# Ewenwan/ORB-YGZ-SLAM

Hardware: AMD Instinct MI355X
Metric: frames/sec ORB-extract+SparseImageAlign, 752x480, 1000 feat (higher is better)
Workload: dtype u8; 1 GPU; C5 offline sequence: 13728 frames (EuRoC MH01..05 length) sharded over 1 GPU(s), per frame C2 extract + dense Hamming (k vs k-1) + C3 SparseImgAlign levels 3..1, device-packed result slots gathered to rank 0 over RCCL; sequence_frames=13728, frames_per_gpu=13728, frames_extracted_per_gpu=13731, chunks=4, image=752x480, nfeatures=1000, nlevels=4, align_pairs_per_gpu=13727, parallelism=frame-sharded x1 (contiguous shards + 1-frame halo), collective=none (N=1: rank 0 is the root), schedule=pipe, hip_graph=False

## Files before the change

orb-ygz-slam_amd/csrc/api_batch.cpp:

```cpp
#include "host.hpp"

namespace ygzfe {
int batch_wait(ygzfe_batch *b) {
    YGZ_HIP(hipStreamSynchronize(b->stream));
    if (b->desc_pending) YGZ_HIP(hipEventSynchronize(b->ev_desc_done));
    return YGZFE_OK;
}
}

static const char *kStageNames[] = {"pyramid", "blur7", "fast9_cells", "octree", "orient_rbrief", "hamming_best2",
                                    "sparse_align", "stereo", "pack_slots"};
constexpr int kNumStages = 9;

extern "C" {

int ygzfe_batch_create(const ygzfe_orb_params *p, int device, int width, int height, int max_frames,
                       ygzfe_batch **out) {
    if (!p || !out || max_frames <= 0) { set_error("invalid argument"); return YGZFE_EINVAL; }
    YGZ_TRY(ensure_device(device));
    std::unique_ptr<ygzfe_batch> b(new ygzfe_batch());
    b->p = *p;
    b->device = device;
    b->maxF = max_frames;
    YGZ_TRY(make_plan(*p, width, height, &b->plan));
    const Plan &P = b->plan->hp();
    YGZ_TRY(b->pyr.ensure((size_t)max_frames * P.pyr_bytes));
    YGZ_TRY(b->ws.ensure(P, max_frames, P.kp_cap));
    YGZ_HIP(hipMemset(b->ws.err.p, 0, 16));
    YGZ_HIP(hipStreamCreateWithFlags(&b->stream, hipStreamNonBlocking));
    for (int i = 0; i < 3; i++) {
        YGZ_HIP(hipStreamCreateWithFlags(&b->aux[i], hipStreamNonBlocking));
        YGZ_HIP(hipEventCreateWithFlags(&b->ev_join[i], hipEventDisableTiming));
    }
    YGZ_HIP(hipEventCreateWithFlags(&b->ev_fork, hipEventDisableTiming));
    YGZ_HIP(hipEventCreateWithFlags(&b->ev_oct_fork, hipEventDisableTiming));
    YGZ_HIP(hipEventCreateWithFlags(&b->ev_desc_done, hipEventDisableTiming));
    for (int i = 0; i < 2; i++) YGZ_HIP(hipEventCreateWithFlags(&b->ev_oct_join[i], hipEventDisableTiming));
    *out = b.release();
    return YGZFE_OK;
}
// ... 41 lines not shown
    YGZ_HIP(hipStreamSynchronize(b->stream));
    if (d_pyramids) b->pyr.bind(d_pyramids, (size_t)b->maxF * P.pyr_bytes);
    if (d_kps) b->ws.kps.bind(d_kps, (size_t)b->maxF * P.kp_cap * sizeof(ygzfe_kp));
    if (d_desc) b->ws.desc.bind(d_desc, (size_t)b->maxF * P.kp_cap * 32);
    if (d_counts) b->ws.counts.bind(d_counts, (size_t)b->maxF * 4);
    return YGZFE_OK;
}

int ygzfe_batch_upload(ygzfe_batch *b, const uint8_t *frames, int n_frames) {
    if (!b || !frames || n_frames < 0 || n_frames > b->maxF) { set_error("invalid argument"); return YGZFE_EINVAL; }
    YGZ_TRY(ensure_device(b->device));
    const Plan &P = b->plan->hp();
    if (b->desc_pending) YGZ_HIP(hipStreamWaitEvent(b->stream, b->ev_desc_done, 0));
    YGZ_HIP(hipMemcpy2DAsync(b->pyr.p, P.pyr_bytes, frames, (size_t)P.W * P.H, (size_t)P.W * P.H, n_frames,
                             hipMemcpyHostToDevice, b->stream));
    YGZ_HIP(hipStreamSynchronize(b->stream));
    return YGZFE_OK;
}

int ygzfe_batch_extract_split(ygzfe_batch *b, int n_frames, void *kp_stream, void *desc_stream) {
    if (!b || n_frames < 0 || n_frames > b->maxF) { set_error("invalid argument"); return YGZFE_EINVAL; }
    if (n_frames == 0) return YGZFE_OK;
    YGZ_TRY(ensure_device(b->device));
    hipStream_t st = kp_stream ? (hipStream_t)kp_stream : b->stream;
    hipStream_t ds = desc_stream ? (hipStream_t)desc_stream : st;
    const PlanDev &pd = *b->plan;
    const Plan &P = pd.hp();
    Workspace &ws = b->ws;
    uint8_t *pyr = b->pyr.as<uint8_t>();
    hipStreamCaptureStatus cap = hipStreamCaptureStatusNone;
    YGZ_HIP(hipStreamIsCapturing(st, &cap));
    if (b->desc_pending && cap == hipStreamCaptureStatusNone) YGZ_HIP(hipStreamWaitEvent(st, b->ev_desc_done, 0));
    YGZ_HIP(hipMemsetAsync(ws.err.p, 0, 16, st));
    static const bool unfused = getenv("YGZFE_PYR_UNFUSED") != nullptr;
    const bool fused = !unfused && pyramid_fusable(P) > 0;
    hipEvent_t t0 = b->begin(st);
    if (fused)
        YGZ_HIP(launch_pyramid_blur0(pyr, ws.blur.as<uint8_t>(), P.pyr_bytes, P, pd.dp(), n_frames, st));
    else
        YGZ_HIP(launch_pyramid(pyr, P.pyr_bytes, P, pd.dp(), pd.tabs.as<int>(), n_frames, st));
    b->end(ST_PYR, t0, st);
    hipStream_t bs = ds;
    if (ds != st) {
        YGZ_HIP(hipEventRecord(b->ev_fork, st));
        YGZ_HIP(hipStreamWaitEvent(ds, b->ev_fork, 0));
    }
    t0 = b->begin(bs);
    if (fused)
        YGZ_HIP(launch_blur_rest(pyr, ws.blur.as<uint8_t>(), P.pyr_bytes, P, pd.dp(), n_frames, bs));
    else
        YGZ_HIP(launch_blur(pyr, ws.blur.as<uint8_t>(), P.pyr_bytes, P, pd.dp(), n_frames, bs));
    b->end(ST_BLUR, t0, bs);
    t0 = b->begin(st);
    YGZ_HIP(launch_fast(pyr, P.pyr_bytes, P, pd.dp(), pd.cells.as<CellDesc>(), ws.cellbuf.as<uint32_t>(),
                        ws.cellcnt.as<int>(), n_frames, st));
    b->end(ST_FAST, t0, st);
    t0 = b->begin(st);
    YGZ_HIP(launch_octree(P, pd.dp(), ws.cellbuf.as<uint32_t>(), ws.cellcnt.as<int>(), ws.candA.as<uint32_t>(),
                          ws.candB.as<uint32_t>(), ws.sel.as<uint32_t>(), ws.selcnt.as<int>(), ws.err.as<int>(),
                          ws.octq.as<int>(),
                          n_frames, st, &b->aux[1], 2, b->ev_oct_fork, b->ev_oct_join));
    YGZ_HIP(launch_emit_kps(P, pd.dp(), ws.sel.as<uint32_t>(), ws.selcnt.as<int>(), nullptr, ws.kps.as<ygzfe_kp>(),
                            ws.counts.as<int>(), P.kp_cap, ws.ojobs.as<uint2>(), n_frames, st));
    b->end(ST_OCT, t0, st);
    if (ds != st) {
        YGZ_HIP(hipEventRecord(b->ev_join[1], st));
        YGZ_HIP(hipStreamWaitEvent(ds, b->ev_join[1], 0));
    }
    t0 = b->begin(ds);
    YGZ_HIP(launch_orient_desc(pyr, ws.blur.as<uint8_t>(), P.pyr_bytes, P, pd.dp(), ws.ojobs.as<uint2>(), nullptr,
                               ws.kps.as<ygzfe_kp>(), ws.desc.as<uint8_t>(), P.kp_cap, n_frames, ds));
    b->end(ST_DESC, t0, ds);
    if (cap == hipStreamCaptureStatusNone) {
        YGZ_HIP(hipEventRecord(b->ev_desc_done, ds));
        b->desc_pending = true;
    }
    return YGZFE_OK;
}

int ygzfe_batch_extract(ygzfe_batch *b, int n_frames, void *stream) {
    return ygzfe_batch_extract_split(b, n_frames, stream, stream);
}

int ygzfe_diag_stage_ms(ygzfe_batch *b, int stage, int n_frames, int reps, int build_pyramid, float *ms) {
    if (!b || !ms || n_frames < 1 || n_frames > b->maxF || reps < 1 || stage < 0 || stage > 2) {
// ... 58 lines not shown
}

int ygzfe_batch_device_results(ygzfe_batch *b, ygzfe_kp **d_kps, uint8_t **d_desc, int32_t **d_counts,
                               int *kp_cap) {
    if (!b) { set_error("null batch"); return YGZFE_EINVAL; }
    if (d_kps) *d_kps = b->ws.kps.as<ygzfe_kp>();
    if (d_desc) *d_desc = b->ws.desc.as<uint8_t>();
    if (d_counts) *d_counts = b->ws.counts.as<int32_t>();
    if (kp_cap) *kp_cap = b->plan->hp().kp_cap;
    return YGZFE_OK;
}

int ygzfe_batch_level(ygzfe_batch *b, int frame, int level, const uint8_t **d_level, int *w, int *h, int *stride) {
    if (!b || frame < 0 || frame >= b->maxF) { set_error("invalid argument"); return YGZFE_EINVAL; }
    const Plan &P = b->plan->hp();
    if (level < 0 || level >= P.nlevels) { set_error("level out of range"); return YGZFE_EINVAL; }
    if (d_level) *d_level = b->pyr.as<uint8_t>() + (size_t)frame * P.pyr_bytes + P.lv[level].off;
    if (w) *w = P.lv[level].w;
    if (h) *h = P.lv[level].h;
    if (stride) *stride = P.lv[level].w;
    return YGZFE_OK;
}

int ygzfe_batch_read_level(ygzfe_batch *b, int frame, int level, int blurred, uint8_t *dst, int dst_stride) {
    if (!b || !dst || frame < 0 || frame >= b->maxF) { set_error("invalid argument"); return YGZFE_EINVAL; }
    const Plan &P = b->plan->hp();
    if (level < 0 || level >= P.nlevels) { set_error("level out of range"); return YGZFE_EINVAL; }
    const LevelDesc &L = P.lv[level];
    if (dst_stride < L.w) { set_error("dst_stride < level width"); return YGZFE_EINVAL; }
    const DevBuf &src = blurred ? b->ws.blur : b->pyr;
    if (!src.p) { set_error("no %s buffer yet (run ygzfe_batch_extract first)", blurred ? "blurred" : "pyramid"); return YGZFE_EINVAL; }
    YGZ_TRY(ensure_device(b->device));
    YGZ_TRY(batch_wait(b));
    YGZ_HIP(hipMemcpy2D(dst, dst_stride, (const uint8_t *)src.p + (size_t)frame * P.pyr_bytes + L.off, L.w, L.w, L.h,
                        hipMemcpyDeviceToHost));
    return YGZFE_OK;
}

int ygzfe_batch_stats(ygzfe_batch *b, int n_frames, int64_t *candidates, int64_t *selected) {
    if (!b || n_frames < 0 || n_frames > b->maxF) { set_error("invalid argument"); return YGZFE_EINVAL; }
    const Plan &P = b->plan->hp();
    YGZ_TRY(ensure_device(b->device));
    YGZ_TRY(batch_wait(b));
    for (int l = 0; l < P.nlevels; l++) {
        if (candidates) candidates[l] = 0;
        if (selected) selected[l] = 0;
    }
    if (n_frames == 0 || !b->ws.cellcnt.p) return YGZFE_OK;
    std::vector<int> cc((size_t)n_frames * P.ncells), sc((size_t)n_frames * P.nlevels);
    if (P.ncells) YGZ_HIP(hipMemcpy(cc.data(), b->ws.cellcnt.p, cc.size() * 4, hipMemcpyDeviceToHost));
    YGZ_HIP(hipMemcpy(sc.data(), b->ws.selcnt.p, sc.size() * 4, hipMemcpyDeviceToHost));
    for (int f = 0; f < n_frames; f++)
        for (int l = 0; l < P.nlevels; l++) {
            const LevelDesc &L = P.lv[l];
            if (candidates)
                for (int c = 0; c < L.ncells; c++) candidates[l] += cc[(size_t)f * P.ncells + L.cell_begin + c];
            if (selected) selected[l] += sc[(size_t)f * P.nlevels + l];
        }
    return YGZFE_OK;
}

int ygzfe_batch_timing(ygzfe_batch *b, int enable, float *ms, const char **names, int cap) {
    if (!b) { set_error("null batch"); return YGZFE_EINVAL; }
    YGZ_TRY(ensure_device(b->device));
    YGZ_TRY(b->collect());
    for (int s = 0; s < kNumStages && s < cap; s++) {
// ... 42 lines not shown
```

orb-ygz-slam_amd/csrc/common.hpp:

```cpp
#pragma once

#include <hip/hip_runtime.h>
#include <stdint.h>

#include "../../include/ygzfe.h"

namespace ygzfe {

constexpr int kMaxLevels = YGZFE_MAX_LEVELS;
#ifndef YGZ_BLUR_ROWS
#define YGZ_BLUR_ROWS 32
#endif
constexpr int kBlurRows = YGZ_BLUR_ROWS;
constexpr int kEdgeThreshold = 19;
constexpr int kMinBorder = kEdgeThreshold - 3;
constexpr int kPatchSize = 31, kHalfPatch = 15;
constexpr int kMaxRoi = 72;

struct LevelDesc {
    int w, h;
    uint32_t off;
    int budget;
    int patch_size;
    float scale, inv_scale;
    int cell_begin, ncells;
    int max_bx, max_by;
    int n_ini;
    float hX;
    int sel_off, sel_cap;
    int cand_off, cand_cap;
    int resize_mode;
    int xtab_off, ytab_off;
    int xmax;
    int blur_tile_begin, blur_tiles_x, blur_tiles_y;
    int pyr_tile_begin;
    int fast_roi;
    int fast_rw, fast_rh;
    int oct_rb, oct_dn, oct_xtab, oct_ytab;
};

struct alignas(16) CellDesc {
    int16_t x0, y0, rw, rh;
    int16_t offx, offy;
    int16_t level, pad;
};

struct Plan {
    int W, H, nlevels;
    uint32_t pyr_bytes;
    int ncells;
    int cell_cap;
    int sel_total;
    int cand_total;
    int kp_cap;
    int ini_th, min_th;
    int blur_variant;
    int blur_tiles;
    int node_cap;
    int fast_S;
    int umax[16];
    LevelDesc lv[kMaxLevels];
    const int32_t *dtabs;
};


template <class T>
using gptr_t = const __attribute__((address_space(1))) T *;
template <class T>
__device__ __forceinline__ gptr_t<T> as_global(const T *p) {
    return (gptr_t<T>)p;
}
template <class T>
using gmut_t = __attribute__((address_space(1))) T *;
template <class T>
__device__ __forceinline__ gmut_t<T> as_global_mut(T *p) {
    return (gmut_t<T>)p;
}
__device__ __forceinline__ uint32_t mad24(uint32_t a, uint32_t b, uint32_t c) {
    uint32_t d;
    asm volatile("v_mad_u32_u24 %0, %1, %2, %3" : "=v"(d) : "v"(a), "v"(b), "v"(c));
    return d;
}

template <class T>
using cptr_t = const __attribute__((address_space(4))) T *;
template <class T>
__device__ __forceinline__ T scalar_load(const T *p) {
    static_assert(sizeof(T) % 4 == 0, "scalar_load: dword-sized records only");
    struct W { uint32_t d[sizeof(T) / 4]; };
    return __builtin_bit_cast(T, *(cptr_t<W>)p);
// ... 180 lines not shown
```

orb-ygz-slam_amd/csrc/extract.hip:

```cpp
#include "common.hpp"

#include <algorithm>
#include <type_traits>

#include "plan.hpp"

namespace ygzfe {

__constant__ __attribute__((aligned(16))) int8_t c_pattern[1024];
__constant__ __attribute__((aligned(16))) uint8_t c_pattern_f8[1024];

#ifdef YGZ_STAMPS
__device__ unsigned long long g_bstamps[1 << 20];
extern "C" int ygzfe_diag_block_stamps(unsigned long long *out, int n) {
    (void)hipDeviceSynchronize();
    (void)hipMemcpyFromSymbol(out, HIP_SYMBOL(g_bstamps), sizeof(unsigned long long) * (size_t)n);
    return 0;
}
#endif


__global__ __launch_bounds__(256) void k_resize_area2(uint8_t *__restrict__ pyr, uint32_t pitch,
                                                      const Plan *__restrict__ plan, int l) {
    const LevelDesc &S = plan->lv[l - 1];
// ... 236 lines not shown
    uint32_t prev;
    uint32_t l1;
    uint32_t l2;
};
#define YGZ_PYR_FUSED_ROW(P, raw, yy, x, store_lane, rs)                                                          \
    do {                                                                                                          \
        if ((yy) & 1) {                                                                                           \
            const uint32_t a_ = __builtin_amdgcn_udot4((raw), 0x00000101u, __builtin_amdgcn_udot4((P).prev, 0x00000101u, 2u, false), false) >> 2; \
            const uint32_t b_ = __builtin_amdgcn_udot4((raw), 0x01010000u, __builtin_amdgcn_udot4((P).prev, 0x01010000u, 2u, false), false) >> 2; \
            if (store_lane)                                                                                       \
                __builtin_amdgcn_raw_buffer_store_b16((uint16_t)(a_ | (b_ << 8)), (rs),                            \
                    (P).off[1] + ((uint32_t)(yy) >> 1) * (P).w[1] + ((uint32_t)(x) >> 1), 0, 0);                   \
            if ((P).K >= 2 && ((yy) & 3) == 3) {                                                                  \
                const uint32_t l2_ = ((P).l1 & 0xFFu) + ((P).l1 >> 8) + a_ + b_ + 2u;                             \
                const uint32_t v2_ = l2_ >> 2;                                                                    \
                if (store_lane)                                                                                   \
                    __builtin_amdgcn_raw_buffer_store_b8((uint8_t)v2_, (rs),                                       \
                        (P).off[2] + ((uint32_t)(yy) >> 2) * (P).w[2] + ((uint32_t)(x) >> 2), 0, 0);               \
                if ((P).K >= 3 && ((yy) & 7) == 7) {                                                              \
                    const uint32_t t_ = (P).l2 + v2_;                                                             \
                    const uint32_t n_ = (uint32_t)__builtin_amdgcn_update_dpp(0, (int)t_, 0xB1, 0xF, 0xF, false); \
                    if ((store_lane) && ((x) & 7) == 0)                                                           \
                        __builtin_amdgcn_raw_buffer_store_b8((uint8_t)((t_ + n_ + 2u) >> 2), (rs),                 \
                            (P).off[3] + ((uint32_t)(yy) >> 3) * (P).w[3] + ((uint32_t)(x) >> 3), 0, 0);           \
                }                                                                                                 \
                (P).l2 = v2_;                                                                                     \
            }                                                                                                     \
            (P).l1 = a_ | (b_ << 8);                                                                              \
        } else {                                                                                                  \
            (P).prev = (raw);                                                                                     \
        }                                                                                                         \
    } while (0)

template <bool CV3, bool PYR>
__device__ __forceinline__ void blur_strip_aligned(const uint8_t *__restrict__ src, uint8_t *__restrict__ dst, int w,
                                                   int hgt, int sx, int y0, int lane, PyrFused &pf) {
    typedef unsigned short u16x2 __attribute__((ext_vector_type(2)));
    constexpr uint32_t k0 = 18, k1 = 34, k2 = CV3 ? 49 : 48, k3 = CV3 ? 55 : 56;
    const int x = sx + 4 * lane;
    const bool left_edge = sx == 0, right_edge = sx + 256 >= w;
    const uint32_t nbytes = (uint32_t)w * (uint32_t)hgt;
    const __amdgpu_buffer_rsrc_t rin = __builtin_amdgcn_make_buffer_rsrc((void *)src, 0, (int)nbytes, 0x00020000);
    const __amdgpu_buffer_rsrc_t rout = __builtin_amdgcn_make_buffer_rsrc((void *)dst, 0, (int)nbytes, 0x00020000);
    const uint32_t voff = (uint32_t)x;
    const uint32_t hoff = lane == 0 ? voff - 4u : voff + 4u;
    constexpr uint32_t K00 = k0 | (k1 << 8) | (k2 << 16) | (k3 << 24), K10 = k2 | (k1 << 8) | (k0 << 16);
    constexpr uint32_t K01 = K00 << 8, K11 = k3 | (k2 << 8) | (k1 << 16) | (k0 << 24);
    constexpr uint32_t K02 = (k0 << 16) | (k1 << 24), K12 = k2 | (k3 << 8) | (k2 << 16) | (k1 << 24), K22 = k0;
    constexpr uint32_t K03 = k0 << 24, K13 = k1 | (k2 << 8) | (k3 << 16) | (k2 << 24), K23 = k1 | (k0 << 8);
    const u16x2 V01 = {(unsigned short)k0, (unsigned short)k1}, V23 = {(unsigned short)k2, (unsigned short)k3};
    const u16x2 V21 = {(unsigned short)k2, (unsigned short)k1};
    struct Row {
        uint32_t a, halo;
    };
    auto fetch = [&](int r, Row &R) {
        const uint32_t so = (uint32_t)(reflect101(y0 + r - 3, hgt) * w);
        R.a = __builtin_amdgcn_raw_buffer_load_b32(rin, voff, so, 0);
        R.halo = __builtin_amdgcn_raw_buffer_load_b32(rin, hoff, so, 0);
    };
    Row buf[kBlurAhead];
#pragma unroll
    for (int r = 0; r < kBlurAhead; r++) fetch(r, buf[r]);
    const bool fix_r = right_edge && x == w;
    const bool fix_halo = right_edge && lane == 63 && w == sx + 256;
    const bool store_lane = x < w;
    uint32_t prv[4] = {0u, 0u, 0u, 0u};
    uint32_t pr[5][4];
    const __amdgpu_buffer_rsrc_t rpyr =
        __builtin_amdgcn_make_buffer_rsrc((void *)pf.frame, 0, PYR ? (int)(pf.off[pf.K] + pf.w[pf.K] * (uint32_t)(hgt >> pf.K)) : 0,
                                          0x00020000);
#pragma unroll
    for (int r = 0; r < kBlurRows + 6; r++) {
        Row cur = buf[r % kBlurAhead];
        if (r + kBlurAhead < kBlurRows + 6) fetch(r + kBlurAhead, buf[r % kBlurAhead]);
        if (PYR && r >= 3 && r < kBlurRows + 3 && y0 + r - 3 < hgt) {
            const int yy = y0 + r - 3;
            YGZ_PYR_FUSED_ROW(pf, cur.a, yy, x, store_lane, rpyr);
        }
        uint32_t am1 = (uint32_t)__builtin_amdgcn_update_dpp((int)cur.halo, (int)cur.a, 0x138, 0xF, 0xF, false);
        if (right_edge) {
            if (fix_r) cur.a = __builtin_amdgcn_perm(cur.a, am1, 0x03000102u);
            if (fix_halo) cur.halo = __builtin_amdgcn_perm(cur.halo, cur.a, 0x03000102u);
        }
        const uint32_t ap1 = (uint32_t)__builtin_amdgcn_update_dpp((int)cur.halo, (int)cur.a, 0x130, 0xF, 0xF, false);
        if (left_edge && lane == 0) am1 = __builtin_amdgcn_perm(ap1, cur.a, 0x01020304u);
        const uint32_t p0 = __builtin_amdgcn_alignbyte(cur.a, am1, 1), p1 = __builtin_amdgcn_alignbyte(ap1, cur.a, 1);
        const uint32_t p2 = ap1 >> 8;
        uint32_t hs[4];
        hs[0] = __builtin_amdgcn_udot4(p1, K10, __builtin_amdgcn_udot4(p0, K00, 0u, false), false);
        hs[1] = __builtin_amdgcn_udot4(p1, K11, __builtin_amdgcn_udot4(p0, K01, 0u, false), false);
        hs[2] = __builtin_amdgcn_udot4(
            p2, K22, __builtin_amdgcn_udot4(p1, K12, __builtin_amdgcn_udot4(p0, K02, 0u, false), false), false);
        hs[3] = __builtin_amdgcn_udot4(
            p2, K23, __builtin_amdgcn_udot4(p1, K13, __builtin_amdgcn_udot4(p0, K03, 0u, false), false), false);
        const int y = y0 + r - 6;
        if (r >= 6 && y < hgt && store_lane) {
            uint32_t pk = 0;
#pragma unroll
            for (int j = 0; j < 4; j++) {
                uint32_t acc = __builtin_amdgcn_udot2(__builtin_bit_cast(u16x2, pr[0][j]), V01, 32768u, false);
                acc = __builtin_amdgcn_udot2(__builtin_bit_cast(u16x2, pr[2][j]), V23, acc, false);
                acc = __builtin_amdgcn_udot2(__builtin_bit_cast(u16x2, pr[4][j]), V21, acc, false);
                uint32_t v = (__umul24(k0, hs[j]) + acc) >> 16;
                if (CV3) v = min(v, 255u);
                pk |= v << (8 * j);
            }
            __builtin_amdgcn_raw_buffer_store_b32(pk, rout, voff, (uint32_t)(y * w), 0);
        }
#pragma unroll
        for (int j = 0; j < 4; j++) {
#pragma unroll
            for (int m = 0; m < 4; m++) pr[m][j] = pr[m + 1][j];
            pr[4][j] = prv[j] | (hs[j] << 16);
            prv[j] = hs[j];
        }
    }
}

#ifndef YGZ_BLUR_EU
#define YGZ_BLUR_EU 7
#endif
#if YGZ_BLUR_EU > 0
#define YGZ_BLUR_ATTR __attribute__((amdgpu_waves_per_eu(YGZ_BLUR_EU)))
#else
#define YGZ_BLUR_ATTR
#endif
template <bool PYR>
__global__ __launch_bounds__(256) YGZ_BLUR_ATTR void k_blur7(uint8_t *__restrict__ pyr,
                                               uint8_t *__restrict__ blur, uint32_t pitch,
                                               const Plan *__restrict__ plan, int task_begin, int task_end,
                                               int pyr_k) {
#ifndef YGZ_BLUR_SWZ
#define YGZ_BLUR_SWZ 1
#endif
    int bx = blockIdx.x, f = blockIdx.y;
    if (YGZ_BLUR_SWZ) swizzled_block_2d(bx, f);
    const int lane = threadIdx.x & 63;
    int task = __builtin_amdgcn_readfirstlane(task_begin + bx * 4 + (threadIdx.x >> 6)), l = 0;
    if (task >= task_end) return;
    while (l + 1 < plan->nlevels && task >= plan->lv[l + 1].blur_tile_begin) l++;
// ... 67 lines not shown
                ring[6][j] = hs[j];
            }
            const int y = y0 + r - 6;
            if (r >= 6 && y < hgt && active) {
                uint32_t pk = 0;
#pragma unroll
                for (int j = 0; j < 4; j++) {
                    const uint32_t acc = __umul24(k0, ring[0][j] + ring[6][j]) + __umul24(k1, ring[1][j] + ring[5][j]) +
                                         __umul24(k2, ring[2][j] + ring[4][j]) + __umul24(k3, ring[3][j]) + 32768u;
                    pk |= min(acc >> 16, 255u) << (8 * j);
                }
                uint8_t *o = dst + (size_t)y * w + x;
                if (x >= 4 && x + 4 <= w - 3 && (((uintptr_t)o) & 3u) == 0) {
                    *reinterpret_cast<uint32_t *>(o) = pk;
                } else {
#pragma unroll
                    for (int j = 0; j < 4; j++)
                        if (x + j >= 4 && x + j < w - 3) o[j] = (uint8_t)(pk >> (8 * j));
                }
            }
        }
    }
    const int ncol = w >= 16 ? 7 : w;
    const bool left = sx == 0, right = sx + 256 >= w;
    if (w >= 16 && !left && !right) return;
    const int nrows = min(kBlurRows, hgt - y0);
    for (int t = lane; t < ncol * nrows; t += 64) {
        const int cidx = t % ncol, r = t / ncol;
        const int xc = w >= 16 ? (cidx < 4 ? cidx : w - 7 + cidx) : cidx;
        if (w >= 16 && ((xc < 4 && !left) || (xc >= w - 3 && !right))) continue;
        const int y = y0 + r;
        dst[(size_t)y * w + xc] = blur_pixel_reflect(src, w, hgt, xc, y, kk);
    }
}


__device__ __forceinline__ int wave_incl_scan(int v) {
    v += __builtin_amdgcn_update_dpp(0, v, 0x111, 0xF, 0xF, false);
    v += __builtin_amdgcn_update_dpp(0, v, 0x112, 0xF, 0xF, false);
    v += __builtin_amdgcn_update_dpp(0, v, 0x114, 0xF, 0xF, false);
    v += __builtin_amdgcn_update_dpp(0, v, 0x118, 0xF, 0xF, false);
    v += __builtin_amdgcn_update_dpp(0, v, 0x142, 0xA, 0xF, false);
    v += __builtin_amdgcn_update_dpp(0, v, 0x143, 0xC, 0xF, false);
    return v;
}

template <int NT>
__device__ __forceinline__ int block_excl_scan(int v, int *red, int *total) {
    const int lane = threadIdx.x & 63, w = threadIdx.x >> 6;
    const int incl = wave_incl_scan(v);
    if (lane == 63) red[w] = incl;
    __syncthreads();
    int off = 0, tot = 0;
#pragma unroll
    for (int i = 0; i < NT / 64; i++) {
        const int r = red[i];
        off += i < w ? r : 0;
        tot += r;
    }
    __syncthreads();
    *total = tot;
    return off + incl - v;
}


template <int S>
// ... 1596 lines not shown
    }
    for (int l = K + 1; l < hp.nlevels; l++) {
        const LevelDesc &D = hp.lv[l];
        dim3 grid((D.w + 63) / 64, (D.h + 3) / 4, nframes);
        if (D.resize_mode == 1)
            hipLaunchKernelGGL(k_resize_area2, grid, dim3(256), 0, st, pyr, pitch, dp, l);
        else
            hipLaunchKernelGGL(k_resize_linear, grid, dim3(256), 0, st, pyr, pitch, dp, dtabs, l);
    }
    return hipGetLastError();
}

hipError_t launch_blur(const uint8_t *pyr, uint8_t *blur, uint32_t pitch, const Plan &hp, const Plan *dp,
                       int nframes, hipStream_t st) {
    hipLaunchKernelGGL(k_blur7<false>, dim3((hp.blur_tiles + 3) / 4, nframes), dim3(256), 0, st,
                       const_cast<uint8_t *>(pyr), blur, pitch, dp, 0, hp.blur_tiles, 0);
    return hipGetLastError();
}

int pyramid_fusable(const Plan &hp) {
    const int K = hp.nlevels - 1;
    if (K < 1 || K > 3 || hp.lv[0].w < 16 || (hp.lv[0].w & 3) || kBlurRows % 8) return 0;
    for (int l = 1; l <= K; l++)
        if (hp.lv[l].resize_mode != 1) return 0;
    return K;
}

hipError_t launch_pyramid_blur0(uint8_t *pyr, uint8_t *blur, uint32_t pitch, const Plan &hp, const Plan *dp,
                                int nframes, hipStream_t st_l0) {
    const int K = pyramid_fusable(hp), n0 = hp.lv[0].blur_tiles_x * hp.lv[0].blur_tiles_y;
    hipLaunchKernelGGL(k_blur7<true>, dim3((n0 + 3) / 4, nframes), dim3(256), 0, st_l0, pyr, blur, pitch, dp, 0, n0, K);
    return hipGetLastError();
}
hipError_t launch_blur_rest(const uint8_t *pyr, uint8_t *blur, uint32_t pitch, const Plan &hp, const Plan *dp,
                            int nframes, hipStream_t st) {
    const int n0 = hp.lv[0].blur_tiles_x * hp.lv[0].blur_tiles_y, n = hp.blur_tiles - n0;
    if (n <= 0) return hipSuccess;
    hipLaunchKernelGGL(k_blur7<false>, dim3((n + 3) / 4, nframes), dim3(256), 0, st, const_cast<uint8_t *>(pyr), blur,
                       pitch, dp, n0, hp.blur_tiles, 0);
    return hipGetLastError();
}

void fast_shape_pick(int rw, int rh, int &S, int &R) {
    fast_slice_shape(rw, rh, S, R);
    if (S == 36 && R > 40) S = 40;
    if (!((S == 36 && R == 40) || (S == 40 && R <= 56))) S = R = std::max(S, R);
}
#define YGZ_FAST_SHAPES(X) X(36, 40) X(40, 40) X(40, 48) X(40, 56) X(48, 48) X(56, 56) X(64, 64) X(72, 72)

hipError_t launch_fast(const uint8_t *pyr, uint32_t pitch, const Plan &hp, const Plan *dp, const CellDesc *dcells,
                       uint32_t *cellbuf, int *cellcnt, int nframes, hipStream_t st0, const hipStream_t *lvl_streams,
                       int n_lvl_streams) {
    if (hp.ncells == 0) return hipSuccess;
    for (int l = 0; l < hp.nlevels; l++) {
        const LevelDesc &L = hp.lv[l];
        if (L.ncells == 0) continue;
        int S, R;
        fast_shape_pick(L.fast_rw, L.fast_rh, S, R);
        const hipStream_t st = (l == 0 || !lvl_streams || n_lvl_streams <= 0) ? st0
                                                                                : lvl_streams[(l - 1) % n_lvl_streams];
#ifndef YGZ_FAST_LDS_MIN
#define YGZ_FAST_LDS_MIN 0
#endif
        const size_t lds = std::max<size_t>(kFastWaves * (size_t)fast_slice_bytes(S, R), YGZ_FAST_LDS_MIN);
        const dim3 grid((L.ncells + kFastWaves - 1) / kFastWaves, nframes);
#define YGZ_FAST(SS, RR)                                                                                        \
    if (S == SS && R == RR)                                                                                     \
        hipLaunchKernelGGL((k_fast_cells<SS, RR>), grid, dim3(64 * kFastWaves), lds, st, pyr, pitch, dp, dcells, \
                           cellbuf, cellcnt, L.cell_begin, L.cell_begin + L.ncells, l, nullptr);
        YGZ_FAST_SHAPES(YGZ_FAST)
#undef YGZ_FAST
    }
// ... 175 lines not shown
```

orb-ygz-slam_amd/csrc/kernels.hpp:

```cpp
#pragma once
#include "common.hpp"

namespace ygzfe {

hipError_t upload_pattern(const int *pat);
hipError_t run_arith_guard(uint32_t host_fails[2]);
hipError_t launch_pyramid(uint8_t *pyr, uint32_t pitch, const Plan &hp, const Plan *dp, const int *dtabs,
                          int nframes, hipStream_t st);
int pyramid_fusable(const Plan &hp);
hipError_t launch_pyramid_blur0(uint8_t *pyr, uint8_t *blur, uint32_t pitch, const Plan &hp, const Plan *dp,
                                int nframes, hipStream_t st_l0);
hipError_t launch_blur_rest(const uint8_t *pyr, uint8_t *blur, uint32_t pitch, const Plan &hp, const Plan *dp,
                            int nframes, hipStream_t st);
hipError_t launch_blur(const uint8_t *pyr, uint8_t *blur, uint32_t pitch, const Plan &hp, const Plan *dp,
                       int nframes, hipStream_t st);
hipError_t launch_fast(const uint8_t *pyr, uint32_t pitch, const Plan &hp, const Plan *dp, const CellDesc *dcells,
                       uint32_t *cellbuf, int *cellcnt, int nframes, hipStream_t st,
                       const hipStream_t *lvl_streams = nullptr, int n_lvl_streams = 0);
hipError_t launch_fast_merged(const uint8_t *pyr, uint32_t pitch, const Plan &hp, const Plan *dp,
                              const CellDesc *dcells, uint32_t *cellbuf, int *cellcnt, int nframes, hipStream_t st,
                              int *clear_flag = nullptr);
hipError_t launch_octree(const Plan &hp, const Plan *dp, const uint32_t *cellbuf, const int *cellcnt,
                         uint32_t *candA, uint32_t *candB, uint32_t *sel, int *selcnt, int *err, int *octq,
                         int nframes, hipStream_t st, const hipStream_t *side = nullptr, int nside = 0,
                         hipEvent_t fork = nullptr, const hipEvent_t *join = nullptr, bool wide = false);
size_t octree_queue_ints(const Plan &hp, int nframes);
void fast_shape_pick(int rw, int rh, int &S, int &R);
void fast_shape_merged(const Plan &hp, int &S, int &R);
int octree_nc(const LevelDesc &L);
int octree_sort0_keys(int nc, bool wide);
int octree_groups(const Plan &hp);
hipError_t launch_emit_kps(const Plan &hp, const Plan *dp, const uint32_t *sel, const int *selcnt,
                           const int *n_existing, ygzfe_kp *kps, int *counts, int row_cap, uint2 *ojobs, int nframes,
                           hipStream_t st);
hipError_t launch_orient_desc(const uint8_t *pyr, const uint8_t *blur, uint32_t pitch, const Plan &hp,
                              const Plan *dp, const uint2 *ojobs, const int *n_existing, ygzfe_kp *kps,
                              uint8_t *desc, int row_cap, int nframes, hipStream_t st);
hipError_t launch_desc_existing(const uint8_t *pyr, const uint8_t *blur, const Plan *dp, ygzfe_kp *kps,
                                uint8_t *desc, int n, int recompute_angle, hipStream_t st);

hipError_t launch_fast10_rois(const uint8_t *img, int stride, const int *rois, int n_rois, int barrier,
                              int variant, int16_t *out_xy, int cap, int *counts, hipStream_t st);
hipError_t launch_dso_occupancy(const ygzfe_kp *kps, int n, uint8_t *occ, int w, int h, hipStream_t st);
hipError_t launch_dso_pass(const uint8_t *img, int w, int h, int g, const uint8_t *occ, uint32_t *keys, int *cnt,
                           hipStream_t st);
hipError_t launch_dso_finish2(const uint32_t *keys, const int *cnt, int ncells, ygzfe_kp *kps, int row0,
// ... 239 lines not shown
```

orb-ygz-slam_amd/csrc/plan.cpp:

```cpp
#include <math.h>
#include <float.h>
#include <string.h>

#include <algorithm>
#include <vector>

#include "plan.hpp"

namespace ygzfe {

static int cv_round_f(float v) { return (int)lrintf(v); }
static int cv_round_d(double v) { return (int)lrint(v); }

void orb_scales(const ygzfe_orb_params &p, ScaleInfo *s) {
    const double sf = (double)p.scale_factor;
    s->scale[0] = 1.0f;
    s->sigma2[0] = 1.0f;
    for (int i = 1; i < p.nlevels; i++) {
        s->scale[i] = (float)((double)s->scale[i - 1] * sf);
        s->sigma2[i] = s->scale[i] * s->scale[i];
    }
    for (int i = 0; i < p.nlevels; i++) {
        s->inv_scale[i] = 1.0f / s->scale[i];
        s->inv_sigma2[i] = 1.0f / s->sigma2[i];
// ... 51 lines not shown
        uint32_t code = 0u;
        for (int d = 1, sh = 32 - rb - 2; d <= Dn; d++, sh -= 2) {
            const int my = y0 + ((y1 - y0 + 1) >> 1);
            const bool by = y >= my;
            (by ? y0 : y1) = my;
            code |= (uint32_t)(by ^ (d & 1)) << (sh + 1);
        }
        tabs->push_back((int)code);
    }
}

int build_plan(const ygzfe_orb_params &p, int W, int H, PlanHost *ph, char *err, size_t errlen) {
    Plan &P = ph->plan;
    memset(&P, 0, sizeof(P));
    ph->cells.clear();
    ph->tabs.clear();
    if (p.nlevels < 1 || p.nlevels > kMaxLevels || p.nfeatures < 0 || !(p.scale_factor > 1.0f) || W < 8 ||
        H < 8) {
        snprintf(err, errlen, "invalid parameters (nlevels=%d nfeatures=%d scale=%g size=%dx%d)", p.nlevels,
                 p.nfeatures, (double)p.scale_factor, W, H);
        return -1;
    }
    ScaleInfo s;
    orb_scales(p, &s);
    ph->scales = s;
    P.W = W;
    P.H = H;
    P.nlevels = p.nlevels;
    P.ini_th = std::min(std::max(p.ini_th_fast, 0), 255);
    P.min_th = std::min(std::max(p.min_th_fast, 0), 255);
    P.blur_variant = p.blur_variant;
    for (int i = 0; i < 16; i++) P.umax[i] = s.umax[i];
    uint32_t off = 0;
    int cell_cap = 1, sel_total = 0, cand_total = 0, blur_tiles = 0, node_need = 0;
    for (int l = 0; l < p.nlevels; l++) {
        LevelDesc &L = P.lv[l];
        L.w = cv_round_f((float)W * s.inv_scale[l]);
        L.h = cv_round_f((float)H * s.inv_scale[l]);
        if (L.w >= 4096 || L.h >= 4096 || L.w < 1 || L.h < 1) {
            snprintf(err, errlen, "level %d size %dx%d outside the supported 1..4095", l, L.w, L.h);
            return -1;
        }
        L.off = off;
        off += (uint32_t)L.w * (uint32_t)L.h;
        off = (off + 15u) & ~15u;
        L.budget = s.budget[l];
        L.patch_size = (int)(kPatchSize * s.scale[l]);
        L.scale = s.scale[l];
        L.inv_scale = s.inv_scale[l];
        L.blur_tile_begin = blur_tiles;
        L.blur_tiles_x = (L.w + 255) / 256;
        L.blur_tiles_y = (L.h + kBlurRows - 1) / kBlurRows;
        blur_tiles += L.blur_tiles_x * L.blur_tiles_y;
        if (l > 0) {
            const LevelDesc &S = P.lv[l - 1];
            const double inv_sx = (double)L.w / S.w, inv_sy = (double)L.h / S.h;
            const double sx = 1. / inv_sx, sy = 1. / inv_sy;
            const int isx = (int)lrint(sx), isy = (int)lrint(sy);
            const bool area_fast = fabs(sx - isx) < DBL_EPSILON && fabs(sy - isy) < DBL_EPSILON;
            if (area_fast && isx == 2 && isy == 2) {
                L.resize_mode = 1;
            } else {
                L.resize_mode = 2;
                L.xtab_off = (int)ph->tabs.size();
                L.xmax = L.w;
                for (int dx = 0; dx < L.w; dx++) {
                    float fx = (float)((dx + 0.5) * sx - 0.5);
                    int ix = (int)floorf(fx);
                    fx -= ix;
                    if (ix < 0) fx = 0, ix = 0;
                    if (ix + 1 >= S.w) {
                        if (dx < L.xmax) L.xmax = dx;
                        if (ix >= S.w - 1) fx = 0, ix = S.w - 1;
                    }
                    const int a0 = std::min(std::max(cv_round_f((1.f - fx) * 2048), -32768), 32767);
                    const int a1 = std::min(std::max(cv_round_f(fx * 2048), -32768), 32767);
                    ph->tabs.push_back(ix);
                    ph->tabs.push_back((int)(((uint32_t)(uint16_t)a0) | ((uint32_t)(uint16_t)a1 << 16)));
                }
                L.ytab_off = (int)ph->tabs.size();
                for (int dy = 0; dy < L.h; dy++) {
                    float fy = (float)((dy + 0.5) * sy - 0.5);
                    int iy = (int)floorf(fy);
                    fy -= iy;
                    const int b0 = std::min(std::max(cv_round_f((1.f - fy) * 2048), -32768), 32767);
                    const int b1 = std::min(std::max(cv_round_f(fy * 2048), -32768), 32767);
// ... 16 lines not shown
                const float iniY = (float)(minB + i * hCell);
                float maxY = iniY + hCell + 6;
                if (iniY >= maxBY - 3) continue;
                if (maxY > maxBY) maxY = (float)maxBY;
                for (int j = 0; j < nCols; j++) {
                    const float iniX = (float)(minB + j * wCell);
                    float maxX = iniX + wCell + 6;
                    if (iniX >= maxBX - 6) continue;
                    if (maxX > maxBX) maxX = (float)maxBX;
                    CellDesc c;
                    c.x0 = (int16_t)(int)iniX;
                    c.y0 = (int16_t)(int)iniY;
                    c.rw = (int16_t)((int)maxX - (int)iniX);
                    c.rh = (int16_t)((int)maxY - (int)iniY);
                    c.offx = (int16_t)(j * wCell);
                    c.offy = (int16_t)(i * hCell);
                    c.level = (int16_t)l;
                    c.pad = 0;
                    if (c.rw > kMaxRoi || c.rh > kMaxRoi) {
                        snprintf(err, errlen, "FAST cell ROI %dx%d exceeds %d", c.rw, c.rh, kMaxRoi);
                        return -1;
                    }
                    const int iw = std::max(c.rw - 6, 0), ih = std::max(c.rh - 6, 0);
                    cell_cap = std::max(cell_cap, ((iw + 1) / 2) * ((ih + 1) / 2));
                    P.fast_S = std::max(P.fast_S, ((std::max((int)c.rw, (int)c.rh) + 3) / 4) * 4);
                    L.fast_roi = std::max(L.fast_roi, std::max((int)c.rw, (int)c.rh));
                    L.fast_rw = std::max(L.fast_rw, (int)c.rw);
                    L.fast_rh = std::max(L.fast_rh, (int)c.rh);
                    ph->cells.push_back(c);
                }
            }
        }
        L.ncells = (int)ph->cells.size() - L.cell_begin;
        const bool has_area = maxBX - minB > 0 && maxBY - minB > 0;
        int nIni = has_area ? (int)roundf((float)(maxBX - minB) / (maxBY - minB)) : 1;
        if (nIni < 1) nIni = 1;
        if (nIni > 8) {
            snprintf(err, errlen, "level %d aspect ratio needs %d initial octree nodes (max 8)", l, nIni);
            return -1;
        }
        L.n_ini = nIni;
        if (has_area) {
            L.hX = (float)(maxBX - minB) / nIni;
            octree_code_tables(L, &ph->tabs);
        } else {
            L.hX = 1.f;
            L.oct_rb = 0;
            L.oct_dn = 3;
            L.oct_xtab = L.oct_ytab = (int)ph->tabs.size();
        }
        L.sel_cap = std::max(L.budget + 4, 4 * nIni + 4) + 8;
        L.sel_off = sel_total;
        sel_total += L.sel_cap;
        node_need = std::max(node_need, L.budget + 4 * nIni + 16);
    }
    for (int l = 0; l < p.nlevels; l++) {
        LevelDesc &L = P.lv[l];
        L.cand_cap = std::max(L.ncells * cell_cap, 1);
        L.cand_off = cand_total;
        cand_total += L.cand_cap;
    }
    P.pyr_bytes = off + 64;
    P.fast_S = std::max(P.fast_S, 8);
    P.ncells = (int)ph->cells.size();
    P.cell_cap = cell_cap;
    P.sel_total = sel_total;
    P.cand_total = cand_total;
    P.kp_cap = sel_total;
    P.blur_tiles = blur_tiles;
    if (node_need <= 512) P.node_cap = 512;
    else if (node_need <= 1024) P.node_cap = 1024;
    else if (node_need <= 2048) P.node_cap = 2048;
    else {
        snprintf(err, errlen, "per-level feature budget too large for the octree node pool (need %d > 2048)",
                 node_need);
        return -1;
    }
    if (ph->tabs.empty()) ph->tabs.push_back(0);
    return 0;
}

}
```

Measured before the change: 571,700 frames/s.

## Pack narrow pyramid levels into sub-wave blur bands and skip unused levels

Adds a banded blur kernel that splits each 64-lane wave into several 16/32-lane bands, so small pyramid levels whose width is far below 256 pixels no longer leave most lanes idle. The plan picks, per level, the band width that needs the fewest waves. Levels with no FAST cells are no longer blurred during extraction; a blurred readback of such a level now blurs it on demand. This cuts wasted lanes and skipped-level work in the blur-rest stage, at the cost of extra edge-handling logic and a lazy blur path on host reads.

```diff
diff --git a/orb-ygz-slam_amd/csrc/api_batch.cpp b/orb-ygz-slam_amd/csrc/api_batch.cpp
--- a/orb-ygz-slam_amd/csrc/api_batch.cpp
+++ b/orb-ygz-slam_amd/csrc/api_batch.cpp
@@ -6,6 +6,11 @@
     if (b->desc_pending) YGZ_HIP(hipEventSynchronize(b->ev_desc_done));
     return YGZFE_OK;
 }
+}
+
+static bool batch_fused(const Plan &P) {
+    static const bool unfused = getenv("YGZFE_PYR_UNFUSED") != nullptr;
+    return !unfused && pyramid_fusable(P) > 0;
 }
 
 static const char *kStageNames[] = {"pyramid", "blur7", "fast9_cells", "octree", "orient_rbrief", "hamming_best2",
@@ -113,8 +118,7 @@
     YGZ_HIP(hipStreamIsCapturing(st, &cap));
     if (b->desc_pending && cap == hipStreamCaptureStatusNone) YGZ_HIP(hipStreamWaitEvent(st, b->ev_desc_done, 0));
     YGZ_HIP(hipMemsetAsync(ws.err.p, 0, 16, st));
-    static const bool unfused = getenv("YGZFE_PYR_UNFUSED") != nullptr;
-    const bool fused = !unfused && pyramid_fusable(P) > 0;
+    const bool fused = batch_fused(P);
     hipEvent_t t0 = b->begin(st);
     if (fused)
         YGZ_HIP(launch_pyramid_blur0(pyr, ws.blur.as<uint8_t>(), P.pyr_bytes, P, pd.dp(), n_frames, st));
@@ -126,12 +130,15 @@
         YGZ_HIP(hipEventRecord(b->ev_fork, st));
         YGZ_HIP(hipStreamWaitEvent(ds, b->ev_fork, 0));
     }
-    t0 = b->begin(bs);
-    if (fused)
+    if (!fused) {
+        t0 = b->begin(bs);
+        YGZ_HIP(launch_blur(pyr, ws.blur.as<uint8_t>(), P.pyr_bytes, P, pd.dp(), n_frames, bs));
+        b->end(ST_BLUR, t0, bs);
+    } else if (!blur_rest_empty(P)) {
+        t0 = b->begin(bs);
         YGZ_HIP(launch_blur_rest(pyr, ws.blur.as<uint8_t>(), P.pyr_bytes, P, pd.dp(), n_frames, bs));
-    else
-        YGZ_HIP(launch_blur(pyr, ws.blur.as<uint8_t>(), P.pyr_bytes, P, pd.dp(), n_frames, bs));
-    b->end(ST_BLUR, t0, bs);
+        b->end(ST_BLUR, t0, bs);
+    }
     t0 = b->begin(st);
     YGZ_HIP(launch_fast(pyr, P.pyr_bytes, P, pd.dp(), pd.cells.as<CellDesc>(), ws.cellbuf.as<uint32_t>(),
                         ws.cellcnt.as<int>(), n_frames, st));
@@ -256,6 +263,12 @@
     if (!src.p) { set_error("no %s buffer yet (run ygzfe_batch_extract first)", blurred ? "blurred" : "pyramid"); return YGZFE_EINVAL; }
     YGZ_TRY(ensure_device(b->device));
     YGZ_TRY(batch_wait(b));
+    if (blurred && batch_fused(P) && blur_rest_skips(P, level)) {
+        if (!b->pyr.p) { set_error("no pyramid buffer yet (run ygzfe_batch_extract first)"); return YGZFE_EINVAL; }
+        YGZ_HIP(launch_blur_level(b->pyr.as<uint8_t>(), b->ws.blur.as<uint8_t>(), P.pyr_bytes, P, b->plan->dp(), frame,
+                                  level, b->stream));
+        YGZ_HIP(hipStreamSynchronize(b->stream));
+    }
     YGZ_HIP(hipMemcpy2D(dst, dst_stride, (const uint8_t *)src.p + (size_t)frame * P.pyr_bytes + L.off, L.w, L.w, L.h,
                         hipMemcpyDeviceToHost));
     return YGZFE_OK;
diff --git a/orb-ygz-slam_amd/csrc/common.hpp b/orb-ygz-slam_amd/csrc/common.hpp
--- a/orb-ygz-slam_amd/csrc/common.hpp
+++ b/orb-ygz-slam_amd/csrc/common.hpp
@@ -33,6 +33,7 @@
     int xtab_off, ytab_off;
     int xmax;
     int blur_tile_begin, blur_tiles_x, blur_tiles_y;
+    int band_lanes, band_tiles_x, band_tiles_y, band_task_begin;
     int pyr_tile_begin;
     int fast_roi;
     int fast_rw, fast_rh;
@@ -56,6 +57,7 @@
     int ini_th, min_th;
     int blur_variant;
     int blur_tiles;
+    int band_tasks;
     int node_cap;
     int fast_S;
     int umax[16];
diff --git a/orb-ygz-slam_amd/csrc/extract.hip b/orb-ygz-slam_amd/csrc/extract.hip
--- a/orb-ygz-slam_amd/csrc/extract.hip
+++ b/orb-ygz-slam_amd/csrc/extract.hip
@@ -292,18 +292,20 @@
         }                                                                                                         \
     } while (0)
 
-template <bool CV3, bool PYR>
+template <bool CV3, bool PYR, bool BANDS = false>
 __device__ __forceinline__ void blur_strip_aligned(const uint8_t *__restrict__ src, uint8_t *__restrict__ dst, int w,
-                                                   int hgt, int sx, int y0, int lane, PyrFused &pf) {
+                                                   int hgt, int sx, int y0, int lane, PyrFused &pf, int bl = 64,
+                                                   bool live = true) {
     typedef unsigned short u16x2 __attribute__((ext_vector_type(2)));
     constexpr uint32_t k0 = 18, k1 = 34, k2 = CV3 ? 49 : 48, k3 = CV3 ? 55 : 56;
     const int x = sx + 4 * lane;
-    const bool left_edge = sx == 0, right_edge = sx + 256 >= w;
+    const bool left_edge = sx == 0, right_edge = sx + 4 * bl >= w;
+    const bool band_first = lane == 0, band_last = lane == bl - 1;
     const uint32_t nbytes = (uint32_t)w * (uint32_t)hgt;
     const __amdgpu_buffer_rsrc_t rin = __builtin_amdgcn_make_buffer_rsrc((void *)src, 0, (int)nbytes, 0x00020000);
     const __amdgpu_buffer_rsrc_t rout = __builtin_amdgcn_make_buffer_rsrc((void *)dst, 0, (int)nbytes, 0x00020000);
     const uint32_t voff = (uint32_t)x;
-    const uint32_t hoff = lane == 0 ? voff - 4u : voff + 4u;
+    const uint32_t hdelta = band_first ? -4u : 4u, hoff = voff + hdelta;
     constexpr uint32_t K00 = k0 | (k1 << 8) | (k2 << 16) | (k3 << 24), K10 = k2 | (k1 << 8) | (k0 << 16);
     constexpr uint32_t K01 = K00 << 8, K11 = k3 | (k2 << 8) | (k1 << 16) | (k0 << 24);
     constexpr uint32_t K02 = (k0 << 16) | (k1 << 24), K12 = k2 | (k3 << 8) | (k2 << 16) | (k1 << 24), K22 = k0;
@@ -314,6 +316,13 @@
         uint32_t a, halo;
     };
     auto fetch = [&](int r, Row &R) {
+        if (BANDS) {
+            const int n = abs(y0 + r - 3);
+            const uint32_t o = mad24((uint32_t)max(min(n, 2 * hgt - 2 - n), 0), (uint32_t)w, voff);
+            R.a = __builtin_amdgcn_raw_buffer_load_b32(rin, o, 0, 0);
+            R.halo = __builtin_amdgcn_raw_buffer_load_b32(rin, o + hdelta, 0, 0);
+            return;
+        }
         const uint32_t so = (uint32_t)(reflect101(y0 + r - 3, hgt) * w);
         R.a = __builtin_amdgcn_raw_buffer_load_b32(rin, voff, so, 0);
         R.halo = __builtin_amdgcn_raw_buffer_load_b32(rin, hoff, so, 0);
@@ -322,8 +331,8 @@
 #pragma unroll
     for (int r = 0; r < kBlurAhead; r++) fetch(r, buf[r]);
     const bool fix_r = right_edge && x == w;
-    const bool fix_halo = right_edge && lane == 63 && w == sx + 256;
-    const bool store_lane = x < w;
+    const bool fix_halo = right_edge && band_last && w == sx + 4 * bl;
+    const bool store_lane = live && x < w;
     uint32_t prv[4] = {0u, 0u, 0u, 0u};
     uint32_t pr[5][4];
     const __amdgpu_buffer_rsrc_t rpyr =
@@ -338,12 +347,14 @@
             YGZ_PYR_FUSED_ROW(pf, cur.a, yy, x, store_lane, rpyr);
         }
         uint32_t am1 = (uint32_t)__builtin_amdgcn_update_dpp((int)cur.halo, (int)cur.a, 0x138, 0xF, 0xF, false);
+        if (BANDS && band_first) am1 = cur.halo;
         if (right_edge) {
             if (fix_r) cur.a = __builtin_amdgcn_perm(cur.a, am1, 0x03000102u);
             if (fix_halo) cur.halo = __builtin_amdgcn_perm(cur.halo, cur.a, 0x03000102u);
         }
-        const uint32_t ap1 = (uint32_t)__builtin_amdgcn_update_dpp((int)cur.halo, (int)cur.a, 0x130, 0xF, 0xF, false);
-        if (left_edge && lane == 0) am1 = __builtin_amdgcn_perm(ap1, cur.a, 0x01020304u);
+        uint32_t ap1 = (uint32_t)__builtin_amdgcn_update_dpp((int)cur.halo, (int)cur.a, 0x130, 0xF, 0xF, false);
+        if (BANDS && band_last) ap1 = cur.halo;
+        if (left_edge && band_first) am1 = __builtin_amdgcn_perm(ap1, cur.a, 0x01020304u);
         const uint32_t p0 = __builtin_amdgcn_alignbyte(cur.a, am1, 1), p1 = __builtin_amdgcn_alignbyte(ap1, cur.a, 1);
         const uint32_t p2 = ap1 >> 8;
         uint32_t hs[4];
@@ -365,7 +376,8 @@
                 if (CV3) v = min(v, 255u);
                 pk |= v << (8 * j);
             }
-            __builtin_amdgcn_raw_buffer_store_b32(pk, rout, voff, (uint32_t)(y * w), 0);
+            if (BANDS) __builtin_amdgcn_raw_buffer_store_b32(pk, rout, mad24((uint32_t)y, (uint32_t)w, voff), 0, 0);
+            else __builtin_amdgcn_raw_buffer_store_b32(pk, rout, voff, (uint32_t)(y * w), 0);
         }
 #pragma unroll
         for (int j = 0; j < 4; j++) {
@@ -499,6 +511,34 @@
         const int y = y0 + r;
         dst[(size_t)y * w + xc] = blur_pixel_reflect(src, w, hgt, xc, y, kk);
     }
+}
+
+__global__ __launch_bounds__(256) __attribute__((amdgpu_waves_per_eu(6))) void k_blur7_bands(const uint8_t *__restrict__ pyr,
+                                                                   uint8_t *__restrict__ blur, uint32_t pitch,
+                                                                   const Plan *__restrict__ plan, int ntasks) {
+    int bx = blockIdx.x, f = blockIdx.y;
+    if (YGZ_BLUR_SWZ) swizzled_block_2d(bx, f);
+    const int lane = threadIdx.x & 63;
+    int task = __builtin_amdgcn_readfirstlane(bx * 4 + (threadIdx.x >> 6)), l = 0;
+    if (task >= ntasks) return;
+    while (l + 1 < plan->nlevels && task >= plan->lv[l + 1].band_task_begin) l++;
+    const LevelDesc &L = plan->lv[l];
+    const int bl = L.band_lanes, nb = 64 / bl, ntiles = L.band_tiles_x * L.band_tiles_y;
+    int tile = (task - L.band_task_begin) * nb + (lane >> (31 - __builtin_clz(bl)));
+    const bool live = tile < ntiles;
+    if (!live) tile = 0;
+    const int ty = tile / L.band_tiles_x, sx = (tile - ty * L.band_tiles_x) * 4 * bl, y0 = ty * kBlurRows;
+    const uint8_t *src = pyr + (size_t)f * pitch + L.off;
+    uint8_t *dst = blur + (size_t)f * pitch + L.off;
+    PyrFused pf;
+    pf.frame = nullptr;
+    pf.K = 0;
+    pf.prev = pf.l1 = pf.l2 = 0u;
+    for (int k = 0; k < 4; k++) pf.off[k] = pf.w[k] = 0u;
+    if (plan->blur_variant == YGZFE_BLUR_CV3)
+        blur_strip_aligned<true, false, true>(src, dst, L.w, L.h, sx, y0, lane & (bl - 1), pf, bl, live);
+    else
+        blur_strip_aligned<false, false, true>(src, dst, L.w, L.h, sx, y0, lane & (bl - 1), pf, bl, live);
 }
 
 
@@ -2161,12 +2201,35 @@
     hipLaunchKernelGGL(k_blur7<true>, dim3((n0 + 3) / 4, nframes), dim3(256), 0, st_l0, pyr, blur, pitch, dp, 0, n0, K);
     return hipGetLastError();
 }
+bool blur_rest_skips(const Plan &hp, int l) { return l > 0 && hp.lv[l].ncells == 0; }
+bool blur_rest_empty(const Plan &hp) {
+    for (int l = 1; l < hp.nlevels; l++)
+        if (!blur_rest_skips(hp, l)) return false;
+    return true;
+}
 hipError_t launch_blur_rest(const uint8_t *pyr, uint8_t *blur, uint32_t pitch, const Plan &hp, const Plan *dp,
                             int nframes, hipStream_t st) {
-    const int n0 = hp.lv[0].blur_tiles_x * hp.lv[0].blur_tiles_y, n = hp.blur_tiles - n0;
-    if (n <= 0) return hipSuccess;
-    hipLaunchKernelGGL(k_blur7<false>, dim3((n + 3) / 4, nframes), dim3(256), 0, st, const_cast<uint8_t *>(pyr), blur,
-                       pitch, dp, n0, hp.blur_tiles, 0);
+    if (hp.band_tasks > 0)
+        hipLaunchKernelGGL(k_blur7_bands, dim3((hp.band_tasks + 3) / 4, nframes), dim3(256), 0, st, pyr, blur, pitch, dp,
+                           hp.band_tasks);
+    for (int l = 1; l < hp.nlevels; l++) {
+        if (blur_rest_skips(hp, l) || hp.lv[l].band_lanes) continue;
+        int e = l;
+        while (e + 1 < hp.nlevels && !blur_rest_skips(hp, e + 1) && !hp.lv[e + 1].band_lanes) e++;
+        const int t0 = hp.lv[l].blur_tile_begin, t1 = e + 1 < hp.nlevels ? hp.lv[e + 1].blur_tile_begin : hp.blur_tiles;
+        hipLaunchKernelGGL(k_blur7<false>, dim3((t1 - t0 + 3) / 4, nframes), dim3(256), 0, st,
+                           const_cast<uint8_t *>(pyr), blur, pitch, dp, t0, t1, 0);
+        l = e;
+    }
+    return hipGetLastError();
+}
+hipError_t launch_blur_level(const uint8_t *pyr, uint8_t *blur, uint32_t pitch, const Plan &hp, const Plan *dp,
+                             int frame, int level, hipStream_t st) {
+    const LevelDesc &L = hp.lv[level];
+    const int n = L.blur_tiles_x * L.blur_tiles_y;
+    hipLaunchKernelGGL(k_blur7<false>, dim3((n + 3) / 4, 1), dim3(256), 0, st,
+                       const_cast<uint8_t *>(pyr) + (size_t)frame * pitch, blur + (size_t)frame * pitch, pitch, dp,
+                       L.blur_tile_begin, L.blur_tile_begin + n, 0);
     return hipGetLastError();
 }
 
diff --git a/orb-ygz-slam_amd/csrc/kernels.hpp b/orb-ygz-slam_amd/csrc/kernels.hpp
--- a/orb-ygz-slam_amd/csrc/kernels.hpp
+++ b/orb-ygz-slam_amd/csrc/kernels.hpp
@@ -12,6 +12,10 @@
                                 int nframes, hipStream_t st_l0);
 hipError_t launch_blur_rest(const uint8_t *pyr, uint8_t *blur, uint32_t pitch, const Plan &hp, const Plan *dp,
                             int nframes, hipStream_t st);
+bool blur_rest_skips(const Plan &hp, int level);
+bool blur_rest_empty(const Plan &hp);
+hipError_t launch_blur_level(const uint8_t *pyr, uint8_t *blur, uint32_t pitch, const Plan &hp, const Plan *dp,
+                             int frame, int level, hipStream_t st);
 hipError_t launch_blur(const uint8_t *pyr, uint8_t *blur, uint32_t pitch, const Plan &hp, const Plan *dp,
                        int nframes, hipStream_t st);
 hipError_t launch_fast(const uint8_t *pyr, uint32_t pitch, const Plan &hp, const Plan *dp, const CellDesc *dcells,
diff --git a/orb-ygz-slam_amd/csrc/plan.cpp b/orb-ygz-slam_amd/csrc/plan.cpp
--- a/orb-ygz-slam_amd/csrc/plan.cpp
+++ b/orb-ygz-slam_amd/csrc/plan.cpp
@@ -107,7 +107,7 @@
     P.blur_variant = p.blur_variant;
     for (int i = 0; i < 16; i++) P.umax[i] = s.umax[i];
     uint32_t off = 0;
-    int cell_cap = 1, sel_total = 0, cand_total = 0, blur_tiles = 0, node_need = 0;
+    int cell_cap = 1, sel_total = 0, cand_total = 0, blur_tiles = 0, band_tasks = 0, node_need = 0;
     for (int l = 0; l < p.nlevels; l++) {
         LevelDesc &L = P.lv[l];
         L.w = cv_round_f((float)W * s.inv_scale[l]);
@@ -127,6 +127,7 @@
         L.blur_tiles_x = (L.w + 255) / 256;
         L.blur_tiles_y = (L.h + kBlurRows - 1) / kBlurRows;
         blur_tiles += L.blur_tiles_x * L.blur_tiles_y;
+        L.band_task_begin = band_tasks;
         if (l > 0) {
             const LevelDesc &S = P.lv[l - 1];
             const double inv_sx = (double)L.w / S.w, inv_sy = (double)L.h / S.h;
@@ -209,6 +210,21 @@
             }
         }
         L.ncells = (int)ph->cells.size() - L.cell_begin;
+        if (l > 0 && L.ncells > 0 && L.w >= 16 && (L.w & 3) == 0 && L.h >= 4) {
+            const int dwords = L.w / 4;
+            int best = 0;
+            for (int bl = 64; bl >= 16; bl >>= 1) {
+                const int tx = (dwords + bl - 1) / bl, per = 64 / bl;
+                const int waves = (tx * L.blur_tiles_y + per - 1) / per;
+                if (!best || waves < best) {
+                    best = waves;
+                    L.band_lanes = bl;
+                    L.band_tiles_x = tx;
+                }
+            }
+            L.band_tiles_y = L.blur_tiles_y;
+            band_tasks += best;
+        }
         const bool has_area = maxBX - minB > 0 && maxBY - minB > 0;
         int nIni = has_area ? (int)roundf((float)(maxBX - minB) / (maxBY - minB)) : 1;
         if (nIni < 1) nIni = 1;
@@ -245,6 +261,7 @@
     P.cand_total = cand_total;
     P.kp_cap = sel_total;
     P.blur_tiles = blur_tiles;
+    P.band_tasks = band_tasks;
     if (node_need <= 512) P.node_cap = 512;
     else if (node_need <= 1024) P.node_cap = 1024;
     else if (node_need <= 2048) P.node_cap = 2048;
```

Result: no change. 572,200 frames/s (median of 6 runs) (+0.1%).
